# yilunliao/vit-search

Measured on AMD Instinct MI355X. Metric: images/sec/node ViT-ResNAS-Tiny supernet train, bs128/GPU, 1/2/4/8 MI355X, higher is better.
Workload: dtype bf16

## Files before the change

### include/vitres_hip.h

```cpp
#ifndef VITRES_HIP_H
#define VITRES_HIP_H

#include <stddef.h>
#include <stdint.h>

#ifdef __cplusplus
extern "C" {
#endif

typedef struct ihipStream_t* vr_stream_t;

#define VR_F32 0
#define VR_BF16 1
#define VR_F16 2

int vr_version(void);

typedef struct vr_rowmap {
    int32_t rpi, rps, off;
} vr_rowmap;

typedef struct vr_gemm_args {
    const void* A;
    const void* B;
// ... 21 lines not shown
    int32_t sched;
    vr_rowmap a_map;
    vr_rowmap b_map;
    vr_rowmap c_map;
    int32_t m_groups;
    void* ws;
    int64_t ws_bytes;
    int32_t ring;
    int32_t k_shares;
    const float* sr_x;
    const int32_t* keep_out;
    const float* tok_src;
    const float* tok_pos;
    int32_t sr_g, sr_cin, sr_tokens;
    int32_t tok_rows, tok_ld, tok_rps, tok_cols;
    int32_t reserved0;
} vr_gemm_args;

int vr_gemm_ws_bytes(void);

int vr_gemm(const vr_gemm_args* args, vr_stream_t stream);

int vr_gemm_group(const vr_gemm_args* args, int32_t count, vr_stream_t stream);

typedef struct vr_ln_epilogue {
    int32_t mode;
    float eps;
    const float* w;
    const float* b;
    const int32_t* keep;
// ... 169 lines not shown
    int32_t flip;
    int32_t reserved[3];
} vr_resample_box;
int vr_resample_u8(const uint8_t* src , const vr_resample_box* boxes ,
                   uint8_t* out , int32_t B, int32_t C, int32_t Hs, int32_t Ws,
                   int32_t So_h, int32_t So_w, int32_t filter ,
                   void* workspace, size_t ws_bytes, vr_stream_t stream);
size_t vr_resample_ws_bytes(int32_t B, int32_t So_h, int32_t So_w);
int vr_resample_band_rows(int32_t C, int32_t Hs, int32_t Ws, int32_t So_h, int32_t So_w, int32_t filter);

int vr_token_mean(const void* y, void* out, int32_t B, int32_t N, int32_t C, int32_t first, int32_t dtype, vr_stream_t stream);
int vr_token_mean_bwd(const void* dmean, void* dy, int32_t B, int32_t N, int32_t C, int32_t first, int32_t dtype,
                      vr_stream_t stream);

int vr_batchsum(const float* in, float* out, int32_t B, int64_t inner, vr_stream_t stream);

int vr_im2col_patch(const float* img, void* col, int32_t B, int32_t Cin, int32_t H, int32_t W, int32_t P,
                    int32_t ldk, int32_t dtype, vr_stream_t stream);
int vr_im2col_patch_map(const float* img, void* col, const int64_t* sample_map, int32_t B, int32_t Cin, int32_t H, int32_t W,
                        int32_t P, int32_t ldk, int32_t dtype, vr_stream_t stream);

int vr_embed_cls(const float* tokens, const float* pos, float* x, const int32_t* keep, int32_t B, int32_t N,
                 int32_t C, int32_t num_tokens, vr_stream_t stream);

int vr_sr_im2col(const void* y, void* col, int32_t B, int32_t g, int32_t C, int32_t num_tokens, int32_t dtype, vr_stream_t stream);
int vr_sr_col2im(const void* dcol, void* dy, int32_t B, int32_t g, int32_t C, int32_t num_tokens, int32_t dtype, vr_stream_t stream);
int vr_sr_resid(const float* x, float* out, int32_t B, int32_t g, int32_t Cin, int32_t Cout, int32_t num_tokens, vr_stream_t stream);
int vr_sr_resid_bwd(const float* dout, float* dx, int32_t B, int32_t g, int32_t Cin, int32_t Cout,
                    int32_t accumulate, int32_t num_tokens, vr_stream_t stream);

// ... 58 lines not shown
```

### vit-search_amd/csrc/gemm.hip

```cpp
#include <cstdlib>
#include <type_traits>
#include <utility>

#include "common.h"
#include "../../include/vitres_hip.h"
#include "gemm_shared.h"

bool vr_gemm_nt_launch(const vr_gemm_args& a, hipStream_t stream, int n_cu);
bool vr_gemm_tn_launch(const vr_gemm_args& a, hipStream_t stream, int n_cu);
bool vr_gemm_tn_group_launch(const vr_gemm_args* args, int count, hipStream_t stream, int n_cu);

namespace {
using namespace vr_gemm_shared;

constexpr int LROW = 144;

template <int WR_, int WC_, int MI_, int NI_> struct TileCfg {
    static constexpr int WR = WR_, WC = WC_, MI = MI_, NI = NI_;
    static constexpr int BM = WR * MI * 32, BN = WC * NI * 32, NTHR = WR * WC * 64;
    static constexpr int A_BYTES = BM * LROW, B_BYTES = BN * LROW, BUF_BYTES = A_BYTES + B_BYTES;
};
typedef TileCfg<2, 2, 2, 2> CfgStd;
typedef TileCfg<2, 4, 4, 2> CfgBig;

// ... 696 lines not shown
    } else {
        if ((a.M * esz) % 4 || (a.lda * esz) % 4 || ((uintptr_t)a.A & 3)) return VR_EALIGN;
    }
    if (!a.b_trans) {
        if (a.ldb % epc || a.ldb < kpad || ((uintptr_t)a.B & 15)) return VR_EALIGN;
    } else {
        if ((a.N * esz) % 4 || (a.ldb * esz) % 4 || ((uintptr_t)a.B & 3)) return VR_EALIGN;
    }
    if (((uintptr_t)a.C & 15) || (a.C2 && ((uintptr_t)a.C2 & 15)) || (a.resid && ((uintptr_t)a.resid & 15)) ||
        (a.bias && ((uintptr_t)a.bias & 15)) || (a.pos && ((uintptr_t)a.pos & 15)) ||
        (a.dact_u && ((uintptr_t)a.dact_u & 15)))
        return VR_EALIGN;
    if (a.in_dtype == VR_F32 && a.out_dtype != VR_F32) return VR_EUNSUPPORTED;
    if (a.in_dtype == VR_F16 && (a.k_shares > 1 || (a.sched & 0x200000))) return VR_EUNSUPPORTED;
    if (a.ws && (((uintptr_t)a.ws & 15) || a.ws_bytes < 0)) return VR_EALIGN;
    return VR_OK;
}

extern "C" int vr_gemm_ws_bytes(void) { return (int)(4096 * 4 + (size_t)cu_count() * 2 * (256 * 128) * sizeof(float)); }

static int fold_validate(const vr_gemm_args& a) {
    if (!a.sr_x && !a.keep_out && a.tok_rows <= 0) return 0;
    if (a.tok_rows < 0) return VR_EINVAL;
    if (a.a_trans || a.b_trans || a.atomic || a.act || a.dact_u || a.C2 || a.out_dtype != VR_F32 || a.in_dtype == VR_F32 || a.N % 8 ||
        a.ldc % 8 || a.n_period > 0 || a.rows_in <= 0 || (a.keep_out && a.keep_n))
        return VR_EUNSUPPORTED;
    if (a.sr_x) {
        const int go = a.sr_g / 2;
        if (a.sr_g <= 0 || (a.sr_g & 1) || a.sr_tokens < 0 || a.rows_in != go * go) return VR_EINVAL;
        if (a.sr_cin <= 0 || a.sr_cin % 8 || a.sr_cin > a.N || a.resid || a.scale) return VR_EUNSUPPORTED;
// ... 14 lines not shown
    vr_gemm_args a = *args;
    const int vrc = gemm_validate(a);
    if (vrc != VR_OK) return vrc;
    const int frc = fold_validate(a);
    if (frc < 0) return frc;
    if (!(a.sched & 4) && vr_gemm_nt_launch(a, (hipStream_t)stream, cu_count())) {
        VR_CHECK_LAUNCH();
        return VR_OK;
    }
    if (frc > 0) return VR_EUNSUPPORTED;
    if (!(a.sched & 4) && vr_gemm_tn_launch(a, (hipStream_t)stream, cu_count())) {
        VR_CHECK_LAUNCH();
        return VR_OK;
    }
    if (a.atomic == 2) return VR_EUNSUPPORTED;
    if ((a.sched & 0x80000) && a.m_groups > 1 && (a.keep_k || (a.a_trans && a.keep_n))) return VR_EUNSUPPORTED;
    if (a.in_dtype == VR_BF16) return launch<bf16_t>(a, (hipStream_t)stream);
    if (a.in_dtype == VR_F16) return launch<f16_t>(a, (hipStream_t)stream);
    return launch<float>(a, (hipStream_t)stream);
}

bool vr_gemm_ntk_launch(const vr_gemm_args& a, hipStream_t stream, int n_cu, const vr_ln_epilogue* ln);

extern "C" int vr_gemm_ln_fold(const vr_gemm_args* args, const vr_ln_epilogue* ln, vr_stream_t stream) {
    if (!args || !ln) return VR_EINVAL;
    vr_gemm_args a = *args;
    const int vrc = gemm_validate(a);
    if (vrc != VR_OK) return vrc;
    if (a.in_dtype != VR_BF16 || a.a_trans || a.atomic || a.split_k > 1 || a.bias_grad || a.pos) return VR_EUNSUPPORTED;
    if (((uintptr_t)ln->y & 15) || ((uintptr_t)ln->w & 15) || ((uintptr_t)ln->b & 15)) return VR_EALIGN;
// ... 28 lines not shown
```

### vit-search_amd/csrc/gemm_tn.hip

```cpp
#include "common.h"
#include "../../include/vitres_hip.h"
#include "gemm_shared.h"

namespace vr_gemm_tn {
using namespace vr_gemm_shared;

typedef __bf16 bfv8 __attribute__((ext_vector_type(8)));
typedef short s4 __attribute__((ext_vector_type(4)));
typedef short s8 __attribute__((ext_vector_type(8)));
typedef __attribute__((address_space(3))) void lds_void;
typedef __attribute__((address_space(3))) s4 lds_s4;
typedef __attribute__((address_space(1))) const void glb_void;

#ifndef TN_CAP10
#define TN_CAP10 20
#endif
constexpr int BT = 64, NTHR = 256;

__device__ const uint4 zero_chunk[4] = {{0, 0, 0, 0}, {0, 0, 0, 0}, {0, 0, 0, 0}, {0, 0, 0, 0}};

template <int TW> struct Geo {
    static constexpr int ROWB = TW * 2, SLOTS = TW / 8, TPP = 1024 / ROWB, PIECES = BT / TPP, PPW = PIECES / 4;
    static constexpr int TILE_BYTES = BT * ROWB;
    static constexpr int F = TW / 32;
// ... 158 lines not shown
            else asm volatile("s_waitcnt vmcnt(0)" ::: "memory");
            __builtin_amdgcn_s_barrier();
            if (kt + 2 < ntiles) issue(kt + 2, buf == 0 ? 2 : buf - 1);
            compute(buf);
            buf = buf == 2 ? 0 : buf + 1;
        }
    }

    if (dbg == 1) {
        if (acc[0][0][0] == 12345.678f) reinterpret_cast<float*>(p.C)[0] = 1.f;
        return;
    }
    float* C = reinterpret_cast<float*>(p.C);
    const RowMap cm = {p.c_map.rpi, p.c_map.rps, p.c_map.off};
    const bool skipz = !store && !(p.sched & 0x8000);
    bool ncol[F];
#pragma unroll
    for (int j = 0; j < F; ++j) {
        const int n = n0 + wn * (TW / 2) + 16 * j + li;
        ncol[j] = n < p.N && (!skipz || kept_col(n, p.n_period, nmax));
    }
#pragma unroll
    for (int i = 0; i < F; ++i)
#pragma unroll
        for (int r = 0; r < 4; ++r) {
            const int m = m0 + wm * (TW / 2) + 16 * i + 4 * g + r;
            if (m >= p.M) continue;
            if (skipz && !kept_col(m, p.k_period, kmax)) continue;
            float* crow = C + map_row(cm, m) * (long long)p.ldc;
#pragma unroll
            for (int j = 0; j < F; ++j) {
                const int n = n0 + wn * (TW / 2) + 16 * j + li;
                if (ncol[j]) {
                    if (store) crow[n] = acc[i][j][r];
                    else atomicAdd(crow + n, acc[i][j][r]);
                }
            }
            if (want_bg && li == 0) {
                if (store) p.bias_grad[m] = accb[i][r];
                else atomicAdd(p.bias_grad + m, accb[i][r]);
            }
        }
}

template <bool BIAS, bool MAPPED, int TW, int STAGES>
__global__ __launch_bounds__(NTHR, 4) void tn_kernel(const vr_gemm_args p) {
    tn_body<BIAS, MAPPED, TW, STAGES>(p, blockIdx.x);
}

constexpr int MAXG = 4;
// ... 215 lines not shown
static int group_split(long long split, const vr_gemm_args& a) {
    if (split < 1) split = 1;
    if (!vr_gemm_shared::group_pure(a.K, a.m_groups)) return (int)split;
    if (split < a.m_groups && !needs_pure(a)) return (int)split;
    const long long q = (split + a.m_groups / 2) / a.m_groups;
    return (int)((q < 1 ? 1 : q) * a.m_groups);
}
static bool needs_pure(const vr_gemm_args& a) { return (a.sched & 0x80000) && a.m_groups > 1 && (a.keep_k || a.keep_n); }

bool vr_gemm_tn_group_launch(const vr_gemm_args* args, int count, hipStream_t stream, int n_cu) {
    using namespace vr_gemm_tn;
    if (count < 2 || count > MAXG) return false;
    for (int i = 0; i < count; ++i) {
        const vr_gemm_args& a = args[i];
        if (!tn_covers(a) || a.a_map.rpi != 0 || a.b_map.rpi != 0 || a.split_k > 0) return false;
        if (needs_pure(a) && (a.atomic == 2 || !vr_gemm_shared::group_pure(a.K, a.m_groups))) return false;
    }
    bool all_store = true, any_store = false;
    for (int i = 0; i < count; ++i) {
        all_store = all_store && args[i].atomic == 2;
        any_store = any_store || args[i].atomic == 2;
    }
    TnGroup g;
    g.count = count;
    int next = 0;
    const long long slices = (args[0].K + BT - 1) / BT;
    bool lean_ok = true;
    for (int i = 0; i < count; ++i)
        lean_ok = lean_ok && (long long)args[i].K * args[i].lda * 2 < 0x7ff00000LL && (long long)args[i].K * args[i].ldb * 2 < 0x7ff00000LL;
    bool same_k = true;
// ... 78 lines not shown
```

### vit-search_amd/csrc/misc.hip

```cpp
#include "common.h"
#include "../../include/vitres_hip.h"

namespace {

template <typename TD>
__global__ __launch_bounds__(256) void cast_kernel(const float* __restrict__ src, TD* __restrict__ dst, long long n) {
    const long long stride = (long long)gridDim.x * blockDim.x * 8;
    for (long long i = ((long long)blockIdx.x * blockDim.x + threadIdx.x) * 8; i < n; i += stride) {
        if (i + 8 <= n) {
            const float4 a = *reinterpret_cast<const float4*>(src + i);
            const float4 b = *reinterpret_cast<const float4*>(src + i + 4);
            *reinterpret_cast<uint4*>(dst + i) =
                make_uint4(Half16<TD>::pk(a.x, a.y), Half16<TD>::pk(a.z, a.w), Half16<TD>::pk(b.x, b.y), Half16<TD>::pk(b.z, b.w));
        } else {
            for (long long j = i; j < n; ++j) Elem<TD>::st(dst + j, src[j]);
        }
    }
}

__global__ __launch_bounds__(256) void cast_transpose_kernel(const float* __restrict__ src, bf16_t* __restrict__ dst,
                                                             const vr_tr_desc* __restrict__ descs) {
    __shared__ float tile[64][65];
    const vr_tr_desc d = descs[blockIdx.y];
    const int tc = (d.cols + 63) / 64, tr = (d.rows + 63) / 64;
// ... 320 lines not shown
    const long long i = (long long)blockIdx.x * 256 + threadIdx.x;
    if (i >= inner) return;
    const int b0 = blockIdx.y * bper, b1 = min(B, b0 + bper);
    float s = 0.f;
    int b = b0;
    for (; b + 8 <= b1; b += 8) {
        float v[8];
#pragma unroll
        for (int u = 0; u < 8; ++u) v[u] = in[(long long)(b + u) * inner + i];
        s += ((v[0] + v[1]) + (v[2] + v[3])) + ((v[4] + v[5]) + (v[6] + v[7]));
    }
    for (; b < b1; ++b) s += in[(long long)b * inner + i];
    atomicAdd(out + i, s);
}

template <typename T>
__global__ __launch_bounds__(256) void token_mean_kernel(const T* __restrict__ y, T* __restrict__ out, int N, int C, int first) {
    const int b = blockIdx.x;
    const float inv = 1.0f / (float)(N - first);
    for (int c = threadIdx.x; c < C; c += blockDim.x) {
        float s = 0.f;
        for (int n = first; n < N; ++n) s += Elem<T>::ld(y + ((long long)b * N + n) * C + c);
        Elem<T>::st(out + (long long)b * C + c, s * inv);
    }
}
template <typename T>
__global__ __launch_bounds__(256) void token_mean_bwd_kernel(const T* __restrict__ dmean, T* __restrict__ dy, int N, int C,
                                                             int first) {
    const int n = first + blockIdx.x % (N - first), b = blockIdx.x / (N - first);
    const float inv = 1.0f / (float)(N - first);
// ... 339 lines not shown
    if (dtype == VR_F32)
        hipLaunchKernelGGL((token_mean_bwd_kernel<float>), grid, dim3(256), 0, (hipStream_t)stream, (const float*)dmean, (float*)dy, N, C, first);
    else if (dtype == VR_BF16)
        hipLaunchKernelGGL((token_mean_bwd_kernel<bf16_t>), grid, dim3(256), 0, (hipStream_t)stream, (const bf16_t*)dmean, (bf16_t*)dy, N, C, first);
    else
        return VR_EUNSUPPORTED;
    VR_CHECK_LAUNCH();
    return VR_OK;
}

extern "C" int vr_batchsum(const float* in, float* out, int32_t B, int64_t inner, vr_stream_t stream) {
    if (!in || !out || B <= 0 || inner <= 0) return VR_EINVAL;
    const int bper = B >= 64 ? 16 : (B >= 16 ? 8 : B);
    hipLaunchKernelGGL(batchsum_kernel, dim3((unsigned)((inner + 255) / 256), (unsigned)((B + bper - 1) / bper)), dim3(256), 0,
                       (hipStream_t)stream, in, out, B, (long long)inner, bper);
    VR_CHECK_LAUNCH();
    return VR_OK;
}

extern "C" int vr_im2col_patch(const float* img, void* col, int32_t B, int32_t Cin, int32_t H, int32_t W, int32_t P,
                               int32_t ldk, int32_t dtype, vr_stream_t stream) {
    return vr_im2col_patch_map(img, col, nullptr, B, Cin, H, W, P, ldk, dtype, stream);
}

extern "C" int vr_im2col_patch_map(const float* img, void* col, const int64_t* sample_map, int32_t B, int32_t Cin, int32_t H,
                                   int32_t W, int32_t P, int32_t ldk, int32_t dtype, vr_stream_t stream) {
    if (!img || !col || B <= 0 || P <= 0 || H % P || W % P || ldk < Cin * P * P) return VR_EINVAL;
    const long long* smap = reinterpret_cast<const long long*>(sample_map);
    dim3 grid(B * (H / P));
    const size_t lds = (size_t)Cin * P * W * sizeof(float);
// ... 234 lines not shown
```

### vit-search_amd/vitres/_lib.py

```python
import ctypes
import os
from ctypes import c_float, c_int32, c_int64, c_uint64, c_void_p

_HERE = os.path.dirname(os.path.abspath(__file__))
LIB_PATH = os.environ.get("VITRES_LIB") or os.path.join(os.path.dirname(_HERE), "lib", "libvitres_hip.so")

VR_F32, VR_BF16, VR_F16 = 0, 1, 2


class RowMap(ctypes.Structure):
    _fields_ = [("rpi", c_int32), ("rps", c_int32), ("off", c_int32)]


class GemmArgs(ctypes.Structure):
    _fields_ = [
        ("A", c_void_p), ("B", c_void_p), ("C", c_void_p), ("C2", c_void_p),
        ("bias", c_void_p), ("pos", c_void_p), ("scale", c_void_p), ("keep_n", c_void_p),
        ("resid", c_void_p), ("dact_u", c_void_p), ("keep_k", c_void_p), ("bias_grad", c_void_p),
        ("M", c_int32), ("N", c_int32), ("K", c_int32),
        ("lda", c_int32), ("ldb", c_int32), ("ldc", c_int32), ("ldu", c_int32),
        ("a_trans", c_int32), ("b_trans", c_int32),
        ("in_dtype", c_int32), ("out_dtype", c_int32),
        ("act", c_int32), ("atomic", c_int32), ("split_k", c_int32), ("rows_in", c_int32), ("n_period", c_int32), ("k_period", c_int32), ("sched", c_int32),
        ("a_map", RowMap), ("b_map", RowMap), ("c_map", RowMap), ("m_groups", c_int32),
        ("ws", c_void_p), ("ws_bytes", c_int64), ("ring", c_int32), ("k_shares", c_int32),
        ("sr_x", c_void_p), ("keep_out", c_void_p), ("tok_src", c_void_p), ("tok_pos", c_void_p),
        ("sr_g", c_int32), ("sr_cin", c_int32), ("sr_tokens", c_int32),
        ("tok_rows", c_int32), ("tok_ld", c_int32), ("tok_rps", c_int32), ("tok_cols", c_int32), ("reserved0", c_int32),
    ]


class LnEpilogue(ctypes.Structure):
    _fields_ = [("mode", c_int32), ("eps", c_float), ("w", c_void_p), ("b", c_void_p), ("keep", c_void_p), ("y", c_void_p),
                ("mean", c_void_p), ("rstd", c_void_p), ("x", c_void_p), ("dw", c_void_p), ("db", c_void_p),
                ("gt_out", c_void_p), ("gt_scale", c_void_p), ("gt_keep", c_void_p), ("grad_copies", c_int32)]


MAX_ZERO_RANGES = 24


class ZeroRanges(ctypes.Structure):
    _fields_ = [("lo", c_int64 * MAX_ZERO_RANGES), ("count", c_int64 * MAX_ZERO_RANGES), ("n", c_int32), ("reserved", c_int32)]

# ... 63 lines not shown
    "vr_token_mix": [c_void_p] * 6 + [c_int32] * 11 + [c_float] * 6 + [c_void_p],
    "vr_normalize_u8": [c_void_p, c_void_p] + [c_int32] * 4 + [c_void_p, c_void_p, c_void_p],
    "vr_token_mix_u8": [c_void_p] * 6 + [c_int32] * 11 + [c_float] * 6 + [c_void_p, c_void_p, c_void_p],
    "vr_mixup": [c_void_p] * 5 + [c_int32] * 5 + [c_float, c_float, c_void_p],
    "vr_mixup_u8": [c_void_p] * 5 + [c_int32] * 5 + [c_float, c_float, c_void_p, c_void_p, c_void_p],
    "vr_random_erase": [c_void_p] + [c_int32] * 4 + [c_void_p, c_int32, c_int32, c_uint64, c_uint64, c_void_p],
    "vr_normalize_u8_erase": [c_void_p, c_void_p] + [c_int32] * 4 + [c_void_p, c_void_p, ctypes.POINTER(EraseArgs), c_void_p],
    "vr_token_mix_u8_erase": [c_void_p] * 6 + [c_int32] * 11 + [c_float] * 6 + [c_void_p, c_void_p, ctypes.POINTER(EraseArgs),
                                                                               c_void_p],
    "vr_mixup_u8_erase": [c_void_p] * 5 + [c_int32] * 5 + [c_float, c_float, c_void_p, c_void_p, ctypes.POINTER(EraseArgs), c_void_p],
    "vr_resample_u8": [c_void_p, c_void_p, c_void_p] + [c_int32] * 7 + [c_void_p, ctypes.c_size_t, c_void_p],
    "vr_resample_band_rows": [c_int32] * 6,
    "vr_token_mean": [c_void_p, c_void_p, c_int32, c_int32, c_int32, c_int32, c_int32, c_void_p],
    "vr_token_mean_bwd": [c_void_p, c_void_p, c_int32, c_int32, c_int32, c_int32, c_int32, c_void_p],
    "vr_batchsum": [c_void_p, c_void_p, c_int32, c_int64, c_void_p],
    "vr_im2col_patch": [c_void_p, c_void_p] + [c_int32] * 7 + [c_void_p],
    "vr_im2col_patch_map": [c_void_p, c_void_p, c_void_p] + [c_int32] * 7 + [c_void_p],
    "vr_embed_cls": [c_void_p] * 4 + [c_int32] * 4 + [c_void_p],
    "vr_sr_im2col": [c_void_p, c_void_p] + [c_int32] * 5 + [c_void_p],
    "vr_sr_col2im": [c_void_p, c_void_p] + [c_int32] * 5 + [c_void_p],
    "vr_sr_resid": [c_void_p, c_void_p] + [c_int32] * 5 + [c_void_p],
    "vr_sr_resid_bwd": [c_void_p, c_void_p] + [c_int32] * 6 + [c_void_p],
    "vr_mask_rows": [c_void_p, c_void_p] + [c_int32] * 3 + [c_void_p],
    "vr_zero_ranges": [c_void_p, ctypes.POINTER(ZeroRanges), c_void_p],
    "vr_zero_ranges_gated": [c_void_p, ctypes.POINTER(ZeroRanges), c_void_p, c_void_p],
    "vr_relayout": [c_void_p, c_void_p, c_int32, c_int32, c_int32, c_int64, c_int64, c_int32, c_int32, c_void_p],
    "vr_relayout_add": [c_void_p, c_void_p, c_int32, c_int32, c_int32, c_int64, c_int64, c_void_p],
    "vr_im2col3x3": [c_void_p, c_void_p] + [c_int32] * 8 + [c_void_p],
    "vr_col2im3x3": [c_void_p, c_void_p] + [c_int32] * 5 + [c_void_p],
    "vr_bn_stats": [c_void_p, c_void_p, c_void_p, c_int64, c_int32, c_int32, c_void_p],
# ... 49 lines not shown
```

### vit-search_amd/vitres/functional.py

```python
import os as _os

import torch

from . import kernels as K

OVERLAP = _os.environ.get('VITRES_OVERLAP', '1') != '0'
FUSE_LN = True
FUSE_LN_MAXN = 256
FUSE_LN_FWD_MAXK = 4096
FUSE_SR = True


def _fold_gemm(x, dt):
    return FUSE_SR and x.is_cuda and K.is_fast16(dt)


LN_COPIES = 64
WGRAD_SCHED = 0
_ln_pending = []


def _ln_dst(grads, wk, bk):
    part = grads.get(wk + ".part")
    if part is None:
        return grads[wk], grads[bk], 1
# ... 119 lines not shown
    __slots__ = ("w", "b", "w_c", "ld", "w_t", "ld_t")

    def __init__(self, w, b, w_c, ld, w_t=None, ld_t=0):
        self.w, self.b, self.w_c, self.ld = w, b, w_c, ld
        self.w_t, self.ld_t = w_t, ld_t


def linear_dgrad(dy, W, dx, M, N_in, K_out, lddy, lddx, **kw):
    if W.w_t is not None and lddy % 8 == 0:
        K.gemm(dy, W.w_t, dx, M=M, N=N_in, K=K_out, lda=lddy, ldb=W.ld_t, ldc=lddx, **kw)
    else:
        K.gemm(dy, W.w_c, dx, M=M, N=N_in, K=K_out, lda=lddy, ldb=W.ld, ldc=lddx, b_trans=True, **kw)


def linear_wgrad(dy, x, dw, M, N_out, K_in, lddy, ldx, ldw=None, a_map=None, b_map=None, db=None, keep_rows=None,
                 keep_cols=None, row_period=0, tokens_per_sample=0, sched=0, collect=None, store=False, split=0, m_groups=None):
    kw = dict(M=N_out, N=K_in, K=M, lda=lddy, ldb=ldx, ldc=ldw or K_in, a_trans=True, b_trans=True,
              atomic=(2 if store else True), split_k=(1 if store else split), a_map=a_map, b_map=b_map, bias_grad=db,
              keep_k=keep_rows, keep_n=keep_cols, k_period=row_period, rows_in=tokens_per_sample, sched=sched,
              m_groups=(K.M_GROUPS[0] if m_groups is None else m_groups))
    if collect is not None:
        collect.append((dy, x, dw, kw))
    else:
        K.gemm(dy, x, dw, **kw)


_block_wgrads = []

def flush_wgrads():
    if not _block_wgrads:
        return
    calls = list(_block_wgrads)
    del _block_wgrads[:]
    if not OVERLAP:
        return K.gemm_group(calls)
# ... 170 lines not shown
def sr_bwd(gout, saved, p, grads, cfg, embed_keep, new_keep, gt=None, next_cast=None):
    flush_wgrads()
    x, mean, rstd, y, col = saved
    B, Ni, C = x.shape
    g = cfg["grid"]
    go = g // 2
    P = go * go
    T = cfg.get("tokens", 1)
    No = T + P
    Co = cfg["cout"]
    dt = cfg["dtype"]
    if gt is None:
        gt = K.scale_mask_cast(gout, None, new_keep, No, dt)
    def wgrads():
        linear_wgrad(gt, y, grads["token.w"], B * T, Co, C, Co, C, a_map=(T, No, 0), b_map=(T, Ni, 0), db=grads["token.b"])
        K.batchsum(gout, grads["pos_sum"])
        linear_wgrad(gt, col, grads["reduce.w"], B * P, Co, 9 * C, Co, 9 * C, a_map=(P, No, T), db=grads["reduce.b"],
                     sched=1 if _overlap(gout) else 0)
        if "finish" in grads:
            grads["finish"]()
    if _overlap(gout):
        on_side(wgrads, gt, gout, grads["reduce.w"], grads["pos_sum"], y, col)
    else:
        wgrads()
    dcol = torch.empty((B * P, 9 * C), dtype=dt, device=x.device)
    linear_dgrad(gt, p["reduce"], dcol, B * P, 9 * C, Co, Co, 9 * C, a_map=(P, No, T), rows_in=P)
    dw, db, cp = _ln_dst(grads, "nw", "nb")
    if FUSE_SR and x.is_cuda and dt == torch.bfloat16 and C % 8 == 0 and Co % 4 == 0:
        dy_tok = torch.empty((B * T, C), dtype=dt, device=x.device)
        linear_dgrad(gt, p["token"], dy_tok, B * T, C, Co, Co, C, a_map=(T, No, 0), rows_in=T)
        out = K.ln_bwd_sr(dcol, dy_tok, gout, x, p["nw"], mean, rstd, embed_keep, g, T, dw, db, next_cast=next_cast, copies=cp)
    else:
        dy = torch.empty((B, Ni, C), dtype=dt, device=x.device)
        K.sr_col2im(dcol, dy, B, g, C, T)
        linear_dgrad(gt, p["token"], dy, B * T, C, Co, Co, C, a_map=(T, No, 0), c_map=(T, Ni, 0), rows_in=T)
        gres = K.sr_resid_bwd(gout, B, g, C, Co, T)
        out = K.ln_bwd(dy, x, p["nw"], mean, rstd, embed_keep, Ni, gres, dw, db, next_cast=next_cast, copies=cp)
# ... 26 lines not shown

def embed0_bwd(g, saved, p, grads, cfg, keep, gt=None, wgrad=True, pos=True):
    flush_wgrads()
    (col,) = saved
    B, N, C = g.shape
    T = cfg.get("tokens", 1)
    P = N - T
    dt = cfg["dtype"]
    ldk = p["proj"].ld
    if gt is None:
        gt = K.scale_mask_cast(g, None, keep, N, dt)
    split = 0
    if g.is_cuda and dt == torch.bfloat16:
        split = max(1, -(-(B * P) // (64 * EMBED_WGRAD_SLICES)))
    if wgrad:
        linear_wgrad(gt, col, grads["proj.w"], B * P, C, ldk, C, ldk, a_map=(P, N, T), db=grads["proj.b"], split=split)
    if pos:
        K.batchsum(g, grads["pos"])


def head_fwd(x, p, cfg, keep, with_patch, save, pre=None):
    B, N, C = x.shape
    dt = cfg["dtype"]
    nc = cfg["classes"]
    y, mean, rstd = pre if pre is not None else K.ln_fwd(x, p["nw"], p["nb"], keep, N, cfg["eps"], dt)
    T = cfg.get("tokens", 1)
    cls = torch.empty((B, nc), dtype=torch.float32, device=x.device)
    K.gemm(y, p["cls"].w_c, cls, M=B, N=nc, K=C, lda=C, ldb=p["cls"].ld, ldc=nc, bias=p["cls"].b, a_map=(1, N, 0))
    pat, ym = None, None
    if with_patch == 3:
        pat = torch.empty((B, nc), dtype=torch.float32, device=x.device)
        K.gemm(y, p["dst"].w_c, pat, M=B, N=nc, K=C, lda=C, ldb=p["dst"].ld, ldc=nc, bias=p["dst"].b, a_map=(1, N, 1))
# ... 63 lines not shown
```

### vit-search_amd/vitres/kernels.py

```python
import ctypes

import numpy as np
import torch

from . import _lib
from ._lib import GemmArgs, LnEpilogue, RowMap, VR_BF16, VR_F16, VR_F32

IDENT = (0, 0, 0)

PROFILE = None
PROFILE_ATTN = None
PROFILE_DESC = None


_DTCODES = {torch.float32: VR_F32, torch.bfloat16: VR_BF16, torch.float16: VR_F16}
_DTNAMES = {VR_F32: "f32", VR_BF16: "bf16", VR_F16: "f16"}


def _dtcode(dtype):
    code = _DTCODES.get(dtype)
    if code is None:
        raise TypeError("unsupported dtype %s (the kernels take float32, bfloat16 or float16)" % dtype)
    return code

# ... 57 lines not shown
WRITE_SKIP = [False]
SKIP_WRITES_BIT = 0x40000
READS_SKIPPED_BIT = 0x80000


def reads_skipped():
    return READS_SKIPPED_BIT if WRITE_SKIP[0] else 0


DBG_POISON = False


def _gemm_args(a, b, out, *, M, N, K, lda, ldb, ldc, a_trans=False, b_trans=False, out2=None, bias=None, pos=None,
               scale=None, keep_n=None, resid=None, dact_u=None, ldu=0, act=0, atomic=False, split_k=1, rows_in=0,
               a_map=None, b_map=None, c_map=None, bias_grad=None, keep_k=None, n_period=0, k_period=0, sched=0, ws="auto",
               ring=0, k_shares=0, m_groups=None, sr_pool=None, keep_out=None, tok_rows=None):
    args = GemmArgs()
    if sr_pool is not None:
        sx, sg, st = sr_pool
        assert sx.dtype == torch.float32 and sx.is_contiguous() and sx.shape[1] == st + sg * sg
        args.sr_x, args.sr_g, args.sr_cin, args.sr_tokens = _p(sx), sg, sx.shape[-1], st
    args.keep_out = _p(keep_out)
    if tok_rows is not None:
        src, tpos, tn, tld, trps, tcols = tok_rows
        assert src.dtype == torch.float32 and (tpos is None or tpos.dtype == torch.float32)
        args.tok_src, args.tok_pos, args.tok_rows, args.tok_ld, args.tok_rps, args.tok_cols = _p(src), _p(tpos), tn, tld, trps, tcols
    if isinstance(ws, str):
        ws = _workspace(a.device) if (not a_trans and is_fast16(a.dtype) and a.is_cuda and K >= 512 and k_shares != 1) else None
    if ws is not None:
        args.ws, args.ws_bytes = ws.data_ptr(), ws.numel() * ws.element_size()
    args.ring, args.k_shares = ring, (k_shares or (K_SHARES if not a_trans else 0))
    args.A, args.B, args.C, args.C2 = _p(a), _p(b), _p(out), _p(out2)
# ... 109 lines not shown
    sc, kp = next_cast if next_cast is not None else (None, None)
    args = _gemm_args(du, wt, dx, M=M, N=N, K=K, lda=lda, ldb=ldb, ldc=N, resid=dx_in, rows_in=rows_in, keep_k=keep_k,
                      k_period=k_period, sched=sched)
    ln = LnEpilogue()
    ln.mode, ln.eps = 1, 0.0
    ln.w, ln.keep, ln.mean, ln.rstd, ln.x = _p(ln_w), _p(ln_keep), _p(mean), _p(rstd), _p(x)
    ln.dw, ln.db, ln.gt_out, ln.gt_scale, ln.gt_keep = _p(dw), _p(db), _p(gt), _p(sc), _p(kp)
    ln.grad_copies = copies
    _launch_gemm_ln(args, ln, du, M, N, K, rows_in, keep_k, ln_keep, k_period, M * N * (4 + 4 + 4 + 2))
    return dx if next_cast is None else (dx, gt)


def gemm(a, b, out, *, M, N, K, lda, ldb, ldc, a_trans=False, b_trans=False, out2=None, bias=None, pos=None,
         scale=None, keep_n=None, resid=None, dact_u=None, ldu=0, act=0, atomic=False, split_k=1, rows_in=0,
         a_map=None, b_map=None, c_map=None, bias_grad=None, keep_k=None, n_period=0, k_period=0, sched=0, ws="auto",
         ring=0, k_shares=0, m_groups=None, sr_pool=None, keep_out=None, tok_rows=None):
    args = _gemm_args(a, b, out, M=M, N=N, K=K, lda=lda, ldb=ldb, ldc=ldc, a_trans=a_trans, b_trans=b_trans, out2=out2,
                      bias=bias, pos=pos, scale=scale, keep_n=keep_n, resid=resid, dact_u=dact_u, ldu=ldu, act=act,
                      atomic=atomic, split_k=split_k, rows_in=rows_in, a_map=a_map, b_map=b_map, c_map=c_map,
                      bias_grad=bias_grad, keep_k=keep_k, n_period=n_period, k_period=k_period, sched=sched, ws=ws,
                      ring=ring, k_shares=k_shares, m_groups=m_groups, sr_pool=sr_pool, keep_out=keep_out, tok_rows=tok_rows)
    if DBG_POISON and (args.sched & SKIP_WRITES_BIT) and keep_n is not None and not a_trans and resid is None and \
            is_fast16(out.dtype):
        out.fill_(float("nan"))
        if out2 is not None:
            out2.fill_(float("nan"))
    if PROFILE is None:
        _lib.check(_lib.lib().vr_gemm(ctypes.byref(args), _stream()), "vr_gemm")
        return out
    flops, alg_bytes = _gemm_work(a, out, M, N, K, a_trans, rows_in, keep_k, keep_n, k_period, n_period, out2=out2, resid=resid,
                                  dact_u=dact_u, pos=pos, bias=bias, atomic=atomic,
                                  skip_writes=bool(args.sched & SKIP_WRITES_BIT))
    e0, e1 = torch.cuda.Event(enable_timing=True), torch.cuda.Event(enable_timing=True)
    e0.record()
    _lib.check(_lib.lib().vr_gemm(ctypes.byref(args), _stream()), "vr_gemm")
    e1.record()
# ... 327 lines not shown
    out = torch.empty((B, C), dtype=y.dtype, device=y.device)
    _lib.check(_lib.lib().vr_token_mean(_p(y), _p(out), B, N, C, first, _dt(y), _stream()), "vr_token_mean")
    return out


def token_mean_bwd(dmean, dy, first):
    B, N, C = dy.shape
    _lib.check(_lib.lib().vr_token_mean_bwd(_p(dmean), _p(dy), B, N, C, first, _dt(dy), _stream()), "vr_token_mean_bwd")
    return dy


def batchsum(x, out):
    B = x.shape[0]
    inner = x.numel() // B
    _lib.check(_lib.lib().vr_batchsum(_p(x), _p(out), B, inner, _stream()), "vr_batchsum")
    return out


def im2col_patch(img, P, ldk, out_dtype, sample_map=None, out=None):
    B, Cin, H, W = img.shape
    col = out if out is not None else torch.empty((B * (H // P) * (W // P), ldk), dtype=out_dtype, device=img.device)
    _lib.check(_lib.lib().vr_im2col_patch_map(_p(img), _p(col), _p(sample_map), B, Cin, H, W, P, ldk, _dtcode(out_dtype),
                                              _stream()), "vr_im2col_patch_map")
    return col


def embed_cls(tokens, pos, x, keep, num_tokens=1):
    B, N, C = x.shape
    _lib.check(_lib.lib().vr_embed_cls(_p(tokens), _p(pos), _p(x), _p(keep), B, N, C, num_tokens, _stream()), "vr_embed_cls")
    return x
# ... 447 lines not shown
```

### vit-search_amd/vitres/nets/vit_sr_supernet.py

```python
import contextlib

import numpy as np
import torch
import torch.nn as nn

from .. import functional as Fn
from .. import kernels as K
from ..registry import register_model
from .channel_drop import ChannelDrop
from .masked_layer_norm import MaskedLayerNorm
from .patch_conv import PatchConvEmbed, PatchEmbed
from .supernet_blocks import Block

_BLOCK_EMBED_INDEX = 0
_EMBED_CHANNEL = 1
_EMBED_CONV_MID_CHANNELS = 2
_BLOCK_HEAD_INDEX = -1
_HEAD_OUT_CHANNEL = 2
_HEAD_IN_CHANNEL = 1
_BLOCK_TYPE = 0
_TYPE_IS_EMBED = 0
_TYPE_IS_TRANS = 1
_TYPE_IS_HEAD = 2
_TYPE_IS_SR = 3
# ... 968 lines not shown
                _, blk, p, cfg, (ek, ka, km, ko, s1, s2), sa, sm = entry
                grads = {"n1w": gv(blk.norm1.weight), "n1b": gv(blk.norm1.bias), "n2w": gv(blk.norm2.weight),
                         "n2b": gv(blk.norm2.bias), "qkv.w": gv(blk.attn.qkv.weight), "qkv.b": gv(blk.attn.qkv.bias),
                         "proj.w": gv(blk.attn.proj.weight), "proj.b": gv(blk.attn.proj.bias),
                         "fc1.w": gv(blk.mlp.fc1.weight), "fc1.b": gv(blk.mlp.fc1.bias),
                         "fc2.w": gv(blk.mlp.fc2.weight), "fc2.b": gv(blk.mlp.fc2.bias)}
                with_parts(grads, ("n1w", blk.norm1.weight), ("n2w", blk.norm2.weight))
                g, gt = Fn.mlp_branch_bwd(g, sm, p, grads, cfg, ek, km, ko, s2, gt=gt, next_cast=(s1, ko))
                nc = consumer_cast(ti)
                g = Fn.attn_branch_bwd(g, sa, p, grads, cfg, ek, ka, ko, s1, gt=gt, next_cast=nc)
                g, gt = g if nc is not None else (g, None)
            elif kind == "sr":
                _, blk, p, cfg, (ek, nk), sv = entry
                co, ci = blk.patch_reduce.weight.shape[0], blk.patch_reduce.weight.shape[1]
                nt = self.num_tokens
                ztmp = K.zero_(torch.empty(co * 9 * ci + (nt + blk.num_patches) * co, dtype=torch.float32, device=dev))
                wtmp = ztmp[:co * 9 * ci].view(co, 9 * ci)
                ptmp = ztmp[co * 9 * ci:].view(nt + blk.num_patches, co)
                def finish(blk=blk, wtmp=wtmp, ptmp=ptmp, co=co, ci=ci, nt=nt, add=getattr(self, "_acc_add", False)):
                    K.put_grad(wtmp, gv(blk.patch_reduce.weight), co, 9, ci, add=add)
                    if add:
                        K.relayout_add(ptmp[nt:], gv(blk.pos_embed), 1, 1, blk.num_patches * co)
                    else:
                        gv(blk.pos_embed).copy_(ptmp[nt:].unsqueeze(0))
                grads = {"nw": gv(blk.norm.weight), "nb": gv(blk.norm.bias), "token.w": gv(blk.token_transform.weight),
                         "token.b": gv(blk.token_transform.bias), "reduce.b": gv(blk.patch_reduce.bias),
                         "reduce.w": wtmp, "pos_sum": ptmp, "finish": finish}
                with_parts(grads, ("nw", blk.norm.weight))
                nc = consumer_cast(ti)
                g = Fn.sr_bwd(g, sv, p, grads, cfg, ek, nk, gt=gt, next_cast=nc)
                g, gt = g if nc is not None else (g, None)
            elif kind == "embed":
                _, ep, ecfg, sv = entry
                ekeep = plan.k(plan.layers[0]["embed"])
                if self.embed_type == _TYPE_IS_EMBED:
                    w = self.patch_embed.proj.weight
                    ld = ep["proj"].ld
                    k = w.numel() // w.shape[0]
                    wt = gv(w).view(w.shape[0], k) if ld == k else K.zero_(torch.empty((w.shape[0], ld), dtype=torch.float32,
                                                                                        device=dev))
                    grads = {"proj.w": wt, "proj.b": gv(self.patch_embed.proj.bias), "pos": gv(self.pos_embed)}

                    def tail(wgrad=True, pos=True, g=g, sv=sv, ep=ep, grads=grads, ecfg=ecfg, ekeep=ekeep, gt=gt, wt=wt, w=w, k=k, ld=ld,
                             add=getattr(self, "_acc_add", False)):
                        Fn.embed0_bwd(g, sv, ep, grads, ecfg, ekeep, gt=gt, wgrad=wgrad, pos=pos)
                        if wgrad and ld != k:
                            K.put_grad(wt, gv(w), w.shape[0], 1, k, src_ld=ld, add=add)
                        if pos:
                            gv(self.tokens).copy_(gv(self.pos_embed)[:, 0:self.num_tokens, :])
                    if Fn._overlap(g):
                        Fn.flush_wgrads()
                        Fn.on_aux("tail", tail, g, gt, wt, *sv)
                        tail_aux = True
                    else:
                        tail()
                else:
                    from .. import stem
                    stem.embed_conv_bwd(self, g, sv, ep, ecfg, ekeep, gv, gt=gt)
                    gv(self.tokens).copy_(gv(self.pos_embed)[:, 0:self.num_tokens, :])
        if tail_aux:
            Fn.on_aux("tail", Fn.flush_ln_grads)
        else:
            Fn.flush_ln_grads()
# ... 57 lines not shown
```

Before: 18650.

## Write SR/embed weight and pos grads directly into parameter layout

Adds column remapping (tap-interleave and column truncation) to the TN wgrad GEMM epilogue so the SR patch_reduce and patch-embed weight gradients land directly in the parameter grad tensors. It also adds a batchsum_to kernel that writes the pos-embed gradient with an offset and a duplicate lead slice for tokens. Together these remove the zeroed temp buffers, the put_grad relayouts and the pos/token copies in backward. The cost is scattered, strided atomic writes in the epilogue and a restriction to bf16, non-accumulating paths.

Result: slower. 18120 (-2.9%).

```diff
diff --git a/include/vitres_hip.h b/include/vitres_hip.h
--- a/include/vitres_hip.h
+++ b/include/vitres_hip.h
@@ -59,6 +59,8 @@
     const float* tok_pos;
     int32_t sr_g, sr_cin, sr_tokens;
     int32_t tok_rows, tok_ld, tok_rps, tok_cols;
+    int32_t wg_taps;
+    int32_t wg_cols;
     int32_t reserved0;
 } vr_gemm_args;
 
@@ -258,6 +260,8 @@
                       vr_stream_t stream);
 
 int vr_batchsum(const float* in, float* out, int32_t B, int64_t inner, vr_stream_t stream);
+int vr_batchsum_to(const float* in, float* out, float* out_lead, int32_t B, int64_t inner, int64_t skip, int64_t lead,
+                   vr_stream_t stream);
 
 int vr_im2col_patch(const float* img, void* col, int32_t B, int32_t Cin, int32_t H, int32_t W, int32_t P,
                     int32_t ldk, int32_t dtype, vr_stream_t stream);
diff --git a/vit-search_amd/csrc/gemm.hip b/vit-search_amd/csrc/gemm.hip
--- a/vit-search_amd/csrc/gemm.hip
+++ b/vit-search_amd/csrc/gemm.hip
@@ -734,6 +734,12 @@
     if (a.in_dtype == VR_F32 && a.out_dtype != VR_F32) return VR_EUNSUPPORTED;
     if (a.in_dtype == VR_F16 && (a.k_shares > 1 || (a.sched & 0x200000))) return VR_EUNSUPPORTED;
     if (a.ws && (((uintptr_t)a.ws & 15) || a.ws_bytes < 0)) return VR_EALIGN;
+    if (a.wg_taps < 0 || a.wg_cols < 0) return VR_EINVAL;
+    if (a.wg_taps > 0 || a.wg_cols > 0) {
+        if (!(a.a_trans && a.b_trans && a.atomic)) return VR_EINVAL;
+        if (a.wg_cols > a.N || (a.wg_taps > 0 && a.N % a.wg_taps)) return VR_EINVAL;
+        if (a.ldc < (a.wg_cols > 0 ? a.wg_cols : a.N)) return VR_EINVAL;
+    }
     return VR_OK;
 }
 
@@ -778,6 +784,7 @@
         return VR_OK;
     }
     if (a.atomic == 2) return VR_EUNSUPPORTED;
+    if (a.wg_taps > 0 || a.wg_cols > 0) return VR_EUNSUPPORTED;
     if ((a.sched & 0x80000) && a.m_groups > 1 && (a.keep_k || (a.a_trans && a.keep_n))) return VR_EUNSUPPORTED;
     if (a.in_dtype == VR_BF16) return launch<bf16_t>(a, (hipStream_t)stream);
     if (a.in_dtype == VR_F16) return launch<f16_t>(a, (hipStream_t)stream);
diff --git a/vit-search_amd/csrc/gemm_tn.hip b/vit-search_amd/csrc/gemm_tn.hip
--- a/vit-search_amd/csrc/gemm_tn.hip
+++ b/vit-search_amd/csrc/gemm_tn.hip
@@ -196,11 +196,15 @@
     float* C = reinterpret_cast<float*>(p.C);
     const RowMap cm = {p.c_map.rpi, p.c_map.rps, p.c_map.off};
     const bool skipz = !store && !(p.sched & 0x8000);
+    const int taps = p.wg_taps, wci = taps > 0 ? p.N / taps : 1;
+    const int nlim = p.wg_cols > 0 ? min(p.N, p.wg_cols) : p.N;
     bool ncol[F];
+    int ocol[F];
 #pragma unroll
     for (int j = 0; j < F; ++j) {
         const int n = n0 + wn * (TW / 2) + 16 * j + li;
-        ncol[j] = n < p.N && (!skipz || kept_col(n, p.n_period, nmax));
+        ncol[j] = n < nlim && (!skipz || kept_col(n, p.n_period, nmax));
+        ocol[j] = taps > 0 ? (n % wci) * taps + n / wci : n;
     }
 #pragma unroll
     for (int i = 0; i < F; ++i)
@@ -212,10 +216,9 @@
             float* crow = C + map_row(cm, m) * (long long)p.ldc;
 #pragma unroll
             for (int j = 0; j < F; ++j) {
-                const int n = n0 + wn * (TW / 2) + 16 * j + li;
                 if (ncol[j]) {
-                    if (store) crow[n] = acc[i][j][r];
-                    else atomicAdd(crow + n, acc[i][j][r]);
+                    if (store) crow[ocol[j]] = acc[i][j][r];
+                    else atomicAdd(crow + ocol[j], acc[i][j][r]);
                 }
             }
             if (want_bg && li == 0) {
@@ -461,6 +464,7 @@
     for (int i = 0; i < count; ++i) {
         const vr_gemm_args& a = args[i];
         if (!tn_covers(a) || a.a_map.rpi != 0 || a.b_map.rpi != 0 || a.split_k > 0) return false;
+        if (a.wg_taps > 0 || a.wg_cols > 0) return false;
         if (needs_pure(a) && (a.atomic == 2 || !vr_gemm_shared::group_pure(a.K, a.m_groups))) return false;
     }
     bool all_store = true, any_store = false;
diff --git a/vit-search_amd/csrc/misc.hip b/vit-search_amd/csrc/misc.hip
--- a/vit-search_amd/csrc/misc.hip
+++ b/vit-search_amd/csrc/misc.hip
@@ -358,6 +358,27 @@
     atomicAdd(out + i, s);
 }
 
+__global__ __launch_bounds__(256) void batchsum_to_kernel(const float* __restrict__ in, float* __restrict__ out,
+                                                          float* __restrict__ lead_out, int B, long long inner, int bper,
+                                                          long long skip, long long lead) {
+    const long long i = (long long)blockIdx.x * 256 + threadIdx.x;
+    if (i >= inner) return;
+    const bool to_out = out != nullptr && i >= skip, to_lead = lead_out != nullptr && i < lead;
+    if (!to_out && !to_lead) return;
+    const int b0 = blockIdx.y * bper, b1 = min(B, b0 + bper);
+    float s = 0.f;
+    int b = b0;
+    for (; b + 8 <= b1; b += 8) {
+        float v[8];
+#pragma unroll
+        for (int u = 0; u < 8; ++u) v[u] = in[(long long)(b + u) * inner + i];
+        s += ((v[0] + v[1]) + (v[2] + v[3])) + ((v[4] + v[5]) + (v[6] + v[7]));
+    }
+    for (; b < b1; ++b) s += in[(long long)b * inner + i];
+    if (to_out) atomicAdd(out + (i - skip), s);
+    if (to_lead) atomicAdd(lead_out + i, s);
+}
+
 template <typename T>
 __global__ __launch_bounds__(256) void token_mean_kernel(const T* __restrict__ y, T* __restrict__ out, int N, int C, int first) {
     const int b = blockIdx.x;
@@ -727,6 +748,17 @@
     const int bper = B >= 64 ? 16 : (B >= 16 ? 8 : B);
     hipLaunchKernelGGL(batchsum_kernel, dim3((unsigned)((inner + 255) / 256), (unsigned)((B + bper - 1) / bper)), dim3(256), 0,
                        (hipStream_t)stream, in, out, B, (long long)inner, bper);
+    VR_CHECK_LAUNCH();
+    return VR_OK;
+}
+
+extern "C" int vr_batchsum_to(const float* in, float* out, float* out_lead, int32_t B, int64_t inner, int64_t skip, int64_t lead,
+                              vr_stream_t stream) {
+    if (!in || (!out && !out_lead) || B <= 0 || inner <= 0) return VR_EINVAL;
+    if (skip < 0 || skip > inner || lead < 0 || lead > inner || (lead > 0 && !out_lead)) return VR_EINVAL;
+    const int bper = B >= 64 ? 16 : (B >= 16 ? 8 : B);
+    hipLaunchKernelGGL(batchsum_to_kernel, dim3((unsigned)((inner + 255) / 256), (unsigned)((B + bper - 1) / bper)), dim3(256), 0,
+                       (hipStream_t)stream, in, out, out_lead, B, (long long)inner, bper, (long long)skip, (long long)lead);
     VR_CHECK_LAUNCH();
     return VR_OK;
 }
diff --git a/vit-search_amd/vitres/_lib.py b/vit-search_amd/vitres/_lib.py
--- a/vit-search_amd/vitres/_lib.py
+++ b/vit-search_amd/vitres/_lib.py
@@ -26,7 +26,8 @@
         ("ws", c_void_p), ("ws_bytes", c_int64), ("ring", c_int32), ("k_shares", c_int32),
         ("sr_x", c_void_p), ("keep_out", c_void_p), ("tok_src", c_void_p), ("tok_pos", c_void_p),
         ("sr_g", c_int32), ("sr_cin", c_int32), ("sr_tokens", c_int32),
-        ("tok_rows", c_int32), ("tok_ld", c_int32), ("tok_rps", c_int32), ("tok_cols", c_int32), ("reserved0", c_int32),
+        ("tok_rows", c_int32), ("tok_ld", c_int32), ("tok_rps", c_int32), ("tok_cols", c_int32),
+        ("wg_taps", c_int32), ("wg_cols", c_int32), ("reserved0", c_int32),
     ]
 
 
@@ -120,6 +121,7 @@
     "vr_token_mean": [c_void_p, c_void_p, c_int32, c_int32, c_int32, c_int32, c_int32, c_void_p],
     "vr_token_mean_bwd": [c_void_p, c_void_p, c_int32, c_int32, c_int32, c_int32, c_int32, c_void_p],
     "vr_batchsum": [c_void_p, c_void_p, c_int32, c_int64, c_void_p],
+    "vr_batchsum_to": [c_void_p, c_void_p, c_void_p, c_int32, c_int64, c_int64, c_int64, c_void_p],
     "vr_im2col_patch": [c_void_p, c_void_p] + [c_int32] * 7 + [c_void_p],
     "vr_im2col_patch_map": [c_void_p, c_void_p, c_void_p] + [c_int32] * 7 + [c_void_p],
     "vr_embed_cls": [c_void_p] * 4 + [c_int32] * 4 + [c_void_p],
diff --git a/vit-search_amd/vitres/functional.py b/vit-search_amd/vitres/functional.py
--- a/vit-search_amd/vitres/functional.py
+++ b/vit-search_amd/vitres/functional.py
@@ -9,6 +9,11 @@
 FUSE_LN_MAXN = 256
 FUSE_LN_FWD_MAXK = 4096
 FUSE_SR = True
+MAP_WGRAD = True
+
+
+def map_wgrad(dev, dt, *dims):
+    return MAP_WGRAD and dev.type == "cuda" and dt == torch.bfloat16 and all(d % 8 == 0 for d in dims)
 
 
 def _fold_gemm(x, dt):
@@ -158,11 +163,14 @@
 
 
 def linear_wgrad(dy, x, dw, M, N_out, K_in, lddy, ldx, ldw=None, a_map=None, b_map=None, db=None, keep_rows=None,
-                 keep_cols=None, row_period=0, tokens_per_sample=0, sched=0, collect=None, store=False, split=0, m_groups=None):
+                 keep_cols=None, row_period=0, tokens_per_sample=0, sched=0, collect=None, store=False, split=0, m_groups=None,
+                 wg_taps=0, wg_cols=0):
     kw = dict(M=N_out, N=K_in, K=M, lda=lddy, ldb=ldx, ldc=ldw or K_in, a_trans=True, b_trans=True,
               atomic=(2 if store else True), split_k=(1 if store else split), a_map=a_map, b_map=b_map, bias_grad=db,
               keep_k=keep_rows, keep_n=keep_cols, k_period=row_period, rows_in=tokens_per_sample, sched=sched,
               m_groups=(K.M_GROUPS[0] if m_groups is None else m_groups))
+    if wg_taps or wg_cols:
+        kw.update(wg_taps=wg_taps, wg_cols=wg_cols)
     if collect is not None:
         collect.append((dy, x, dw, kw))
     else:
@@ -363,13 +371,16 @@
         gt = K.scale_mask_cast(gout, None, new_keep, No, dt)
     def wgrads():
         linear_wgrad(gt, y, grads["token.w"], B * T, Co, C, Co, C, a_map=(T, No, 0), b_map=(T, Ni, 0), db=grads["token.b"])
-        K.batchsum(gout, grads["pos_sum"])
+        if "pos" in grads:
+            K.batchsum_to(gout, grads["pos"], skip=T * Co)
+        else:
+            K.batchsum(gout, grads["pos_sum"])
         linear_wgrad(gt, col, grads["reduce.w"], B * P, Co, 9 * C, Co, 9 * C, a_map=(P, No, T), db=grads["reduce.b"],
-                     sched=1 if _overlap(gout) else 0)
+                     sched=1 if _overlap(gout) else 0, wg_taps=grads.get("reduce.taps", 0))
         if "finish" in grads:
             grads["finish"]()
     if _overlap(gout):
-        on_side(wgrads, gt, gout, grads["reduce.w"], grads["pos_sum"], y, col)
+        on_side(wgrads, gt, gout, grads["reduce.w"], grads.get("pos_sum"), y, col)
     else:
         wgrads()
     dcol = torch.empty((B * P, 9 * C), dtype=dt, device=x.device)
@@ -426,8 +437,12 @@
     if g.is_cuda and dt == torch.bfloat16:
         split = max(1, -(-(B * P) // (64 * EMBED_WGRAD_SLICES)))
     if wgrad:
-        linear_wgrad(gt, col, grads["proj.w"], B * P, C, ldk, C, ldk, a_map=(P, N, T), db=grads["proj.b"], split=split)
-    if pos:
+        wc = grads.get("proj.cols", 0)
+        linear_wgrad(gt, col, grads["proj.w"], B * P, C, ldk, C, ldk, ldw=wc or ldk, a_map=(P, N, T), db=grads["proj.b"], split=split,
+                     wg_cols=wc)
+    if pos and "tokens" in grads:
+        K.batchsum_to(g, grads["pos"], lead_out=grads["tokens"], lead=T * C)
+    elif pos:
         K.batchsum(g, grads["pos"])
 
 
diff --git a/vit-search_amd/vitres/kernels.py b/vit-search_amd/vitres/kernels.py
--- a/vit-search_amd/vitres/kernels.py
+++ b/vit-search_amd/vitres/kernels.py
@@ -95,8 +95,9 @@
 def _gemm_args(a, b, out, *, M, N, K, lda, ldb, ldc, a_trans=False, b_trans=False, out2=None, bias=None, pos=None,
                scale=None, keep_n=None, resid=None, dact_u=None, ldu=0, act=0, atomic=False, split_k=1, rows_in=0,
                a_map=None, b_map=None, c_map=None, bias_grad=None, keep_k=None, n_period=0, k_period=0, sched=0, ws="auto",
-               ring=0, k_shares=0, m_groups=None, sr_pool=None, keep_out=None, tok_rows=None):
+               ring=0, k_shares=0, m_groups=None, sr_pool=None, keep_out=None, tok_rows=None, wg_taps=0, wg_cols=0):
     args = GemmArgs()
+    args.wg_taps, args.wg_cols = wg_taps, wg_cols
     if sr_pool is not None:
         sx, sg, st = sr_pool
         assert sx.dtype == torch.float32 and sx.is_contiguous() and sx.shape[1] == st + sg * sg
@@ -236,12 +237,13 @@
 def gemm(a, b, out, *, M, N, K, lda, ldb, ldc, a_trans=False, b_trans=False, out2=None, bias=None, pos=None,
          scale=None, keep_n=None, resid=None, dact_u=None, ldu=0, act=0, atomic=False, split_k=1, rows_in=0,
          a_map=None, b_map=None, c_map=None, bias_grad=None, keep_k=None, n_period=0, k_period=0, sched=0, ws="auto",
-         ring=0, k_shares=0, m_groups=None, sr_pool=None, keep_out=None, tok_rows=None):
+         ring=0, k_shares=0, m_groups=None, sr_pool=None, keep_out=None, tok_rows=None, wg_taps=0, wg_cols=0):
     args = _gemm_args(a, b, out, M=M, N=N, K=K, lda=lda, ldb=ldb, ldc=ldc, a_trans=a_trans, b_trans=b_trans, out2=out2,
                       bias=bias, pos=pos, scale=scale, keep_n=keep_n, resid=resid, dact_u=dact_u, ldu=ldu, act=act,
                       atomic=atomic, split_k=split_k, rows_in=rows_in, a_map=a_map, b_map=b_map, c_map=c_map,
                       bias_grad=bias_grad, keep_k=keep_k, n_period=n_period, k_period=k_period, sched=sched, ws=ws,
-                      ring=ring, k_shares=k_shares, m_groups=m_groups, sr_pool=sr_pool, keep_out=keep_out, tok_rows=tok_rows)
+                      ring=ring, k_shares=k_shares, m_groups=m_groups, sr_pool=sr_pool, keep_out=keep_out, tok_rows=tok_rows,
+                      wg_taps=wg_taps, wg_cols=wg_cols)
     if DBG_POISON and (args.sched & SKIP_WRITES_BIT) and keep_n is not None and not a_trans and resid is None and \
             is_fast16(out.dtype):
         out.fill_(float("nan"))
@@ -599,6 +601,15 @@
     B = x.shape[0]
     inner = x.numel() // B
     _lib.check(_lib.lib().vr_batchsum(_p(x), _p(out), B, inner, _stream()), "vr_batchsum")
+    return out
+
+
+def batchsum_to(x, out, skip=0, lead_out=None, lead=0):
+    B = x.shape[0]
+    inner = x.numel() // B
+    assert out is None or out.numel() == inner - skip
+    assert lead_out is None or lead_out.numel() == lead
+    _lib.check(_lib.lib().vr_batchsum_to(_p(x), _p(out), _p(lead_out), B, inner, skip, lead, _stream()), "vr_batchsum_to")
     return out
 
 
diff --git a/vit-search_amd/vitres/nets/vit_sr_supernet.py b/vit-search_amd/vitres/nets/vit_sr_supernet.py
--- a/vit-search_amd/vitres/nets/vit_sr_supernet.py
+++ b/vit-search_amd/vitres/nets/vit_sr_supernet.py
@@ -1006,18 +1006,22 @@
                 _, blk, p, cfg, (ek, nk), sv = entry
                 co, ci = blk.patch_reduce.weight.shape[0], blk.patch_reduce.weight.shape[1]
                 nt = self.num_tokens
-                ztmp = K.zero_(torch.empty(co * 9 * ci + (nt + blk.num_patches) * co, dtype=torch.float32, device=dev))
-                wtmp = ztmp[:co * 9 * ci].view(co, 9 * ci)
-                ptmp = ztmp[co * 9 * ci:].view(nt + blk.num_patches, co)
-                def finish(blk=blk, wtmp=wtmp, ptmp=ptmp, co=co, ci=ci, nt=nt, add=getattr(self, "_acc_add", False)):
-                    K.put_grad(wtmp, gv(blk.patch_reduce.weight), co, 9, ci, add=add)
-                    if add:
-                        K.relayout_add(ptmp[nt:], gv(blk.pos_embed), 1, 1, blk.num_patches * co)
-                    else:
-                        gv(blk.pos_embed).copy_(ptmp[nt:].unsqueeze(0))
                 grads = {"nw": gv(blk.norm.weight), "nb": gv(blk.norm.bias), "token.w": gv(blk.token_transform.weight),
-                         "token.b": gv(blk.token_transform.bias), "reduce.b": gv(blk.patch_reduce.bias),
-                         "reduce.w": wtmp, "pos_sum": ptmp, "finish": finish}
+                         "token.b": gv(blk.token_transform.bias), "reduce.b": gv(blk.patch_reduce.bias)}
+                if not getattr(self, "_acc_add", False) and Fn.map_wgrad(dev, self.compute_dtype, co, ci):
+                    grads.update({"reduce.w": gv(blk.patch_reduce.weight).view(co, ci * 9), "reduce.taps": 9,
+                                  "pos": gv(blk.pos_embed)})
+                else:
+                    ztmp = K.zero_(torch.empty(co * 9 * ci + (nt + blk.num_patches) * co, dtype=torch.float32, device=dev))
+                    wtmp = ztmp[:co * 9 * ci].view(co, 9 * ci)
+                    ptmp = ztmp[co * 9 * ci:].view(nt + blk.num_patches, co)
+                    def finish(blk=blk, wtmp=wtmp, ptmp=ptmp, co=co, ci=ci, nt=nt, add=getattr(self, "_acc_add", False)):
+                        K.put_grad(wtmp, gv(blk.patch_reduce.weight), co, 9, ci, add=add)
+                        if add:
+                            K.relayout_add(ptmp[nt:], gv(blk.pos_embed), 1, 1, blk.num_patches * co)
+                        else:
+                            gv(blk.pos_embed).copy_(ptmp[nt:].unsqueeze(0))
+                    grads.update({"reduce.w": wtmp, "pos_sum": ptmp, "finish": finish})
                 with_parts(grads, ("nw", blk.norm.weight))
                 nc = consumer_cast(ti)
                 g = Fn.sr_bwd(g, sv, p, grads, cfg, ek, nk, gt=gt, next_cast=nc)
@@ -1029,16 +1033,21 @@
                     w = self.patch_embed.proj.weight
                     ld = ep["proj"].ld
                     k = w.numel() // w.shape[0]
-                    wt = gv(w).view(w.shape[0], k) if ld == k else K.zero_(torch.empty((w.shape[0], ld), dtype=torch.float32,
-                                                                                        device=dev))
+                    mapped = not getattr(self, "_acc_add", False) and Fn.map_wgrad(dev, self.compute_dtype, w.shape[0], ld)
+                    wt = gv(w).view(w.shape[0], k) if (ld == k or mapped) else K.zero_(torch.empty((w.shape[0], ld), dtype=torch.float32,
+                                                                                                    device=dev))
                     grads = {"proj.w": wt, "proj.b": gv(self.patch_embed.proj.bias), "pos": gv(self.pos_embed)}
+                    if mapped:
+                        grads["tokens"] = gv(self.tokens)
+                        if ld != k:
+                            grads["proj.cols"] = k
 
                     def tail(wgrad=True, pos=True, g=g, sv=sv, ep=ep, grads=grads, ecfg=ecfg, ekeep=ekeep, gt=gt, wt=wt, w=w, k=k, ld=ld,
-                             add=getattr(self, "_acc_add", False)):
+                             add=getattr(self, "_acc_add", False), mapped=mapped):
                         Fn.embed0_bwd(g, sv, ep, grads, ecfg, ekeep, gt=gt, wgrad=wgrad, pos=pos)
-                        if wgrad and ld != k:
+                        if wgrad and ld != k and not mapped:
                             K.put_grad(wt, gv(w), w.shape[0], 1, k, src_ld=ld, add=add)
-                        if pos:
+                        if pos and not mapped:
                             gv(self.tokens).copy_(gv(self.pos_embed)[:, 0:self.num_tokens, :])
                     if Fn._overlap(g):
                         Fn.flush_wgrads()
```
